# lpylpy0514/VitTracker

Hardware: NVIDIA B200
Metric: tracked frames/sec over B concurrent tracks (higher is better)
Workload: dtype f32

## Files before the change

### vittracker_b200/csrc/vt_block_tc.cu

```cuda
#include "vt_internal.h"
#include "vt_tc.cuh"

namespace vt {

using namespace tc;

#ifdef VT_TC_TRACE
__device__ long long g_tc_trace[2][4096];
__device__ int g_tc_trace_n[2];
#define TC_TRACE(side)                                                                      \
    do {                                                                                    \
        if (blockIdx.x == 0) { int k__ = g_tc_trace_n[side]; if (k__ < 4096) { g_tc_trace[side][k__] = clock64(); g_tc_trace_n[side] = k__ + 1; } } \
    } while (0)
#else
#define TC_TRACE(side) do {} while (0)
#endif

namespace {

#ifndef VT_TC_NS
#define VT_TC_NS 6
#endif
constexpr int kNS = VT_TC_NS;
constexpr int kEpiWarps = 4 * kNS;
constexpr int kEpiThreads = kEpiWarps * 32;
constexpr int kTcThreads = kEpiThreads + 32;
constexpr int kCW = kC / kNS;
constexpr int kQW = 3 * kC / kNS;
constexpr int kHW = kHid / kNS;
static_assert(kNS == 3 || kNS == 6, "column groups");

constexpr uint32_t kColBig = 0;
constexpr uint32_t kColOut = 320;
constexpr uint32_t kColOpa = 368;
constexpr uint32_t kColHA = 0, kColHB = 192;
constexpr uint32_t kColYA = 384, kColYB = 432;

constexpr int kSmWa = 0;
constexpr int kSmX = kSmWa + kTcWaBytes;
constexpr int kKBytes = kN * kC * 2;
constexpr int kSmKhi = kSmX, kSmKlo = kSmX + kKBytes, kSmVhi = kSmX + 2 * kKBytes, kSmVlo = kSmX + 3 * kKBytes;
constexpr int kSmW2hi = kSmX, kSmW2lo = kSmX + 18432;
constexpr int kSmW1 = kSmX + 4 * kKBytes;
constexpr int kSmW1hi = kSmW1, kSmW1lo = kSmW1 + 18432;
constexpr int kSmPar = kSmW1 + 36864;
constexpr int kSmRed = kSmPar + kDepth * kTcParFloats * 4;
constexpr int kSmBar = kSmRed + 6 * kNS * 128 * 4;
constexpr int kSmTmem = kSmBar + 20 * 8;
static_assert(kSmTmem + 16 <= 227 * 1024, "shared memory");
constexpr int kTcSmemBytes = kSmTmem + 16;
static_assert(kTcWbBytes == 2 * 36864 && 36864 <= 4 * kKBytes, "W2 overlays the K/V region");
static_assert(kSmBar % 8 == 0 && kSmX % 128 == 0, "alignment");

constexpr int kPLn1g = 0, kPLn1b = 48, kPBqkv = 96, kPBproj = 240, kPLn2g = 288, kPLn2b = 336, kPBfc1 = 384, kPBfc2 = 576;

__device__ __forceinline__ void epi_bar() { asm volatile("bar.sync 1, %0;" ::"n"(kEpiThreads) : "memory"); }

struct Epi {
    uint32_t tbase;
    uint32_t lane_addr;
    int q, s, lane, row;
    float* red;
    uint64_t *mb_go, *mb_done;
    uint32_t done_ph;

    __device__ __forceinline__ bool active(int t) const { return !(t == 2 && q >= 2); }
    __device__ __forceinline__ uint32_t taddr(uint32_t col) const { return tbase + lane_addr + col; }

    __device__ __forceinline__ void signal(uint64_t* bar, bool wrote_smem) {
        tc_wait_st();
        if (wrote_smem) fence_async_smem();
        tc_fence_before();
        __syncwarp();
        if (lane == 0) mbar_arrive(bar);
    }
    __device__ __forceinline__ void signal_go(bool wrote_smem) { signal(mb_go, wrote_smem); }
    __device__ __forceinline__ void wait_bar(uint64_t* bar, uint32_t& ph) {
        if (threadIdx.x == 0) TC_TRACE(1);
        mbar_wait(bar, ph);
        ph ^= 1;
        tc_fence_after();
        if (threadIdx.x == 0) TC_TRACE(1);
    }
    __device__ __forceinline__ void wait_done() {
        if (threadIdx.x == 0) TC_TRACE(1);
        mbar_wait(mb_done, done_ph);
        done_ph ^= 1;
        tc_fence_after();
        if (threadIdx.x == 0) TC_TRACE(1);
    }

    __device__ __forceinline__ float row_sum(float partial, int arr) {
        float* r = red + arr * (kNS * 128);
        r[s * 128 + row] = partial;
        epi_bar();
        float t = r[row];
#pragma unroll
        for (int g = 1; g < kNS; ++g) t += r[g * 128 + row];
        return t;
    }

    __device__ __forceinline__ void ln(const float (&v)[kCW], const float* g, const float* b, float (&y)[kCW]) {
        float sum = 0.f;
#pragma unroll
        for (int i = 0; i < kCW; ++i) sum += v[i];
        const float mean = row_sum(sum, 0) * (1.f / 48.f);
        float var = 0.f;
#pragma unroll
        for (int i = 0; i < kCW; ++i) { const float d = v[i] - mean; var = fmaf(d, d, var); }
        const float rstd = rsqrtf(row_sum(var, 1) * (1.f / 48.f) + kLnEps);
#pragma unroll
        for (int i = 0; i < kCW; ++i) y[i] = (v[i] - mean) * rstd * g[kCW * s + i] + b[kCW * s + i];
    }

    __device__ __forceinline__ void store_opa(int t, const float (&y)[kCW]) {
        uint32_t hi[kCW / 2], lo[kCW / 2];
#pragma unroll
        for (int j = 0; j < kCW / 2; ++j) split_pack2(y[2 * j], y[2 * j + 1], hi[j], lo[j]);
        tmem_st<kCW / 2>(taddr(kColOpa + 48 * t + (kCW / 2) * s), hi);
        tmem_st<kCW / 2>(taddr(kColOpa + 48 * t + 24 + (kCW / 2) * s), lo);
    }
};

__device__ __forceinline__ float ex2_approx(float x) {
    float y;
    asm("ex2.approx.ftz.f32 %0, %1;" : "=f"(y) : "f"(x));
    return y;
}
__device__ __forceinline__ float rcp_approx(float x) {
    float y;
    asm("rcp.approx.ftz.f32 %0, %1;" : "=f"(y) : "f"(x));
    return y;
}
__device__ __forceinline__ float gelu_erf(float v) {
    const float av = fabsf(v);
    const float t = rcp_approx(fmaf(0.3275911f * 0.70710678118654752f, av, 1.f));
    float p = fmaf(0.5f * 1.061405429f, t, 0.5f * -1.453152027f);
    p = fmaf(p, t, 0.5f * 1.421413741f);
    p = fmaf(p, t, 0.5f * -0.284496736f);
    p = fmaf(p, t, 0.5f * 0.254829592f);
    const float e = ex2_approx(v * (-0.5f * 1.4426950408889634f * v));
    return fmaf(-(av * (p * t)), e, fmaxf(v, 0.f));
}

__device__ __forceinline__ uint64_t f2pack(float lo, float hi) {
    uint64_t r;
    asm("mov.b64 %0, {%1, %2};" : "=l"(r) : "f"(lo), "f"(hi));
    return r;
}
__device__ __forceinline__ void f2unpack(uint64_t v, float& lo, float& hi) { asm("mov.b64 {%0, %1}, %2;" : "=f"(lo), "=f"(hi) : "l"(v)); }
__device__ __forceinline__ uint64_t f2bcast(float c) { return f2pack(c, c); }
__device__ __forceinline__ uint64_t f2fma(uint64_t a, uint64_t b, uint64_t c) {
    uint64_t r;
    asm("fma.rn.f32x2 %0, %1, %2, %3;" : "=l"(r) : "l"(a), "l"(b), "l"(c));
    return r;
}
__device__ __forceinline__ uint64_t f2mul(uint64_t a, uint64_t b) {
    uint64_t r;
    asm("mul.rn.f32x2 %0, %1, %2;" : "=l"(r) : "l"(a), "l"(b));
    return r;
}
__device__ __forceinline__ uint64_t f2add(uint64_t a, uint64_t b) {
    uint64_t r;
    asm("add.rn.f32x2 %0, %1, %2;" : "=l"(r) : "l"(a), "l"(b));
    return r;
}
__device__ __forceinline__ void gelu_erf2(uint64_t v, float& h0, float& h1) {
    float v0, v1;
    f2unpack(v, v0, v1);
    const uint64_t av = f2pack(fabsf(v0), fabsf(v1));
    float d0, d1;
    f2unpack(f2fma(f2bcast(0.3275911f * 0.70710678118654752f), av, f2bcast(1.f)), d0, d1);
    const uint64_t t = f2pack(rcp_approx(d0), rcp_approx(d1));
    uint64_t p = f2fma(f2bcast(-0.5f * 1.061405429f), t, f2bcast(0.5f * 1.453152027f));
    p = f2fma(p, t, f2bcast(-0.5f * 1.421413741f));
    p = f2fma(p, t, f2bcast(0.5f * 0.284496736f));
    p = f2fma(p, t, f2bcast(-0.5f * 0.254829592f));
    float w0, w1;
    f2unpack(f2mul(v, f2mul(f2bcast(-0.5f * 1.4426950408889634f), v)), w0, w1);
    const uint64_t e = f2pack(ex2_approx(w0), ex2_approx(w1));
    f2unpack(f2fma(f2mul(av, f2mul(p, t)), e, f2pack(fmaxf(v0, 0.f), fmaxf(v1, 0.f))), h0, h1);
}

}

template <int kScoresTerms>
__global__ void __launch_bounds__(kTcThreads, 1)
blocks_tc_kernel(const float* __restrict__ tok_z, int z_stride_rows, const float* __restrict__ tok_x, int x_stride_rows,
                 float* __restrict__ out, int n, ModelW w, float* __restrict__ taps, size_t tap_stride) {
    extern __shared__ __align__(128) uint8_t smem[];
    const int tid = threadIdx.x, warp = tid >> 5, lane = tid & 31;
    float* s_par = reinterpret_cast<float*>(smem + kSmPar);
    float* s_red = reinterpret_cast<float*>(smem + kSmRed);
    uint64_t* mb_go = reinterpret_cast<uint64_t*>(smem + kSmBar);
    uint64_t* mb_done = mb_go + 1;
    uint64_t* mb_wa = mb_go + 2;
    uint64_t* mb_wb = mb_go + 3;
    uint64_t* mb_h = mb_go + 4;
    uint64_t* mb_y = mb_go + 6;
    uint64_t* mb_g = mb_go + 8;
    uint64_t* mb_yfree = mb_go + 10;
    uint64_t* mb_w1 = mb_go + 11;
    uint64_t* mb_qd = mb_go + 12;
    uint64_t* mb_pa = mb_go + 15;
    uint64_t* mb_qf = mb_go + 14;
    uint64_t* mb_l1 = mb_go + 16;
    uint32_t* s_tmem = reinterpret_cast<uint32_t*>(smem + kSmTmem);

    if (warp == kEpiWarps) tmem_alloc(s_tmem, 512);
    if (tid == 0) {
        mbar_init(mb_go, kEpiWarps);
        mbar_init(mb_done, 1);
        mbar_init(mb_wa, 1);
        mbar_init(mb_wb, 1);
        mbar_init(mb_w1, 1);
        mbar_init(mb_qd, 1); mbar_init(mb_qd + 1, 1);
        mbar_init(mb_qf, kEpiWarps);
        mbar_init(mb_pa, kEpiWarps);
        for (int t = 0; t < 3; ++t) mbar_init(mb_l1 + t, kEpiWarps);
        mbar_init(mb_h, 1); mbar_init(mb_h + 1, 1);
        mbar_init(mb_y, 1); mbar_init(mb_y + 1, 1);
        mbar_init(mb_g, kEpiWarps); mbar_init(mb_g + 1, kEpiWarps);
        mbar_init(mb_yfree, kEpiWarps);
        mbar_fence_init();
    }
    for (int i = tid; i < kDepth * kTcParFloats; i += kTcThreads) s_par[i] = __ldg(w.tc[i / kTcParFloats].par + i % kTcParFloats);
    tc_fence_before();
    __syncthreads();
    tc_fence_after();
    const uint32_t tbase = __shfl_sync(0xffffffffu, *s_tmem, 0);
    const uint32_t sbase = smem_u32(smem);

    if (warp == kEpiWarps) {
        {
            uint32_t go_ph = 0, wa_ph = 0, wb_ph = 0, w1_ph = 0;
            const uint32_t id48 = instr_desc_f16(128, 48, false), id48mn = instr_desc_f16(128, 48, true);
            const uint32_t id144 = instr_desc_f16(128, 144, false), id160 = instr_desc_f16(128, 160, false);
            const uint32_t id192 = instr_desc_f16(128, 192, false);
            auto wait_go = [&]() { TC_TRACE(0); mbar_wait(mb_go, go_ph); go_ph ^= 1; tc_fence_after(); TC_TRACE(0); };
            auto load_wa = [&](int blk) { bulk_g2s_elect(smem + kSmWa, w.tc[blk].wa, kTcWaBytes, mb_wa); };
            auto load_w1 = [&](int blk) { bulk_g2s_elect(smem + kSmW1, w.tc[blk].wb, 36864, mb_w1); };
            auto load_w2 = [&](int blk) { bulk_g2s_elect(smem + kSmX, w.tc[blk].wb + 36864, 36864, mb_wb); };
            auto gemm_k48 = [&](int t, uint32_t d_col, uint32_t b_hi, uint32_t b_lo, int N, uint32_t idesc) {
                const uint32_t a = tbase + kColOpa + 48 * t;
#pragma unroll
                for (int ks = 0; ks < 3; ++ks) {
                    const uint64_t bh = smem_desc(sbase + b_hi + ks * 2 * N * 16, N * 16, 128);
                    const uint64_t bl = smem_desc(sbase + b_lo + ks * 2 * N * 16, N * 16, 128);
                    mma_ts_elect(tbase + d_col, a + 8 * ks, bh, idesc, ks > 0);
                    mma_ts_elect(tbase + d_col, a + 24 + 8 * ks, bh, idesc, true);
                    mma_ts_elect(tbase + d_col, a + 8 * ks, bl, idesc, true);
                }
            };
            auto qkv = [&](int t, uint32_t d_col) { gemm_k48(t, d_col, kSmWa, kSmWa + 13824, 144, id144); };
            auto fc1 = [&](int t, uint32_t h_col) { gemm_k48(t, h_col, kSmW1hi, kSmW1lo, 192, id192); };
            auto scores_half = [&](int t, int half) {
                const uint32_t a = tbase + kColOpa + 48 * t;
                const uint32_t d = tbase + kColBig + 160 * half;
#pragma unroll
                for (int ks = 0; ks < 3; ++ks) {
                    const uint32_t off = ks * 2 * (kN * 16) + half * 160 * 16;
                    const uint64_t bh = smem_desc(sbase + kSmKhi + off, kN * 16, 128);
                    const uint64_t bl = smem_desc(sbase + kSmKlo + off, kN * 16, 128);
                    mma_ts_elect(d, a + 8 * ks, bh, id160, ks > 0);
                    if (kScoresTerms >= 2) mma_ts_elect(d, a + 24 + 8 * ks, bh, id160, true);
                    if (kScoresTerms >= 3) mma_ts_elect(d, a + 8 * ks, bl, id160, true);
                }
            };
            auto pv = [&](int t, int g0, int g1) {
                const uint32_t d = tbase + kColOpa + 48 * t;
#pragma unroll 5
                for (int g = g0; g < g1; ++g) {
                    const uint32_t a = tbase + kColBig + 16 * g;
                    const uint64_t bh = smem_desc(sbase + kSmVhi + g * 256, 128, (kN / 8) * 128);
                    const uint64_t bl = smem_desc(sbase + kSmVlo + g * 256, 128, (kN / 8) * 128);
                    mma_ts_elect(d, a, bh, id48mn, g > 0);
                    mma_ts_elect(d, a + 8, bh, id48mn, true);
                    mma_ts_elect(d, a, bl, id48mn, true);
                }
            };
            auto fc2 = [&](uint32_t h_col, uint32_t y_col) {
#pragma unroll 4
                for (int g = 0; g < kHid / 16; ++g) {
                    const uint32_t a = tbase + h_col + 16 * g;
                    const uint64_t bh = smem_desc(sbase + kSmW2hi + g * 2 * 48 * 16, 48 * 16, 128);
                    const uint64_t bl = smem_desc(sbase + kSmW2lo + g * 2 * 48 * 16, 48 * 16, 128);
                    mma_ts_elect(tbase + y_col, a, bh, id48, g > 0);
                    mma_ts_elect(tbase + y_col, a + 8, bh, id48, true);
                    mma_ts_elect(tbase + y_col, a, bl, id48, true);
                }
            };
            uint32_t h_ph[2] = {0, 0}, y_ph[2] = {0, 0}, g_ph[2] = {0, 0}, yfree_ph = 0, qf_ph = 0, pa_ph = 0, l1_ph[3] = {0, 0, 0};
            auto wait_on = [&](uint64_t* bar, uint32_t& ph) { TC_TRACE(0); mbar_wait(bar, ph); ph ^= 1; tc_fence_after(); TC_TRACE(0); };
            bool first = true;
            for (int trk = blockIdx.x; trk < n; trk += gridDim.x) {
                const bool last_track = trk + (int)gridDim.x >= n;
                for (int blk = 0; blk < kDepth; ++blk) {
                    if (first) { load_wa(0); load_w1(0); first = false; }
                    wait_on(mb_l1, l1_ph[0]);
                    mbar_wait(mb_wa, wa_ph); wa_ph ^= 1;
                    qkv(0, kColBig); mma_commit_elect(mb_qd);
                    wait_on(mb_l1 + 1, l1_ph[1]); qkv(1, kColBig + 160); mma_commit_elect(mb_qd + 1);
                    wait_on(mb_l1 + 2, l1_ph[2]);
                    wait_on(mb_qf, qf_ph);
                    qkv(2, kColBig); mma_commit_elect(mb_qd);
                    wait_go(); scores_half(0, 0); scores_half(0, 1); mma_commit_elect(mb_done);
#pragma unroll
                    for (int t = 0; t < 3; ++t) {
                        wait_on(mb_pa, pa_ph);
#ifdef VT_TC_LATE_ISSUE
                        wait_go();
                        pv(t, 0, 10);
                        if (t < 2) scores_half(t + 1, 0);
#else
                        pv(t, 0, 10);
                        if (t < 2) scores_half(t + 1, 0);
                        wait_go();
#endif
                        pv(t, 10, 20);
                        if (t < 2) scores_half(t + 1, 1);
                        mma_commit_elect(mb_done);
                    }
                    wait_go(); load_w2(blk);
                    if (!(last_track && blk == kDepth - 1)) load_wa((blk + 1) % kDepth);
                    mbar_wait(mb_w1, w1_ph); w1_ph ^= 1;
                    fc1(0, kColHA); mma_commit_elect(mb_h);
                    wait_on(mb_h, h_ph[0]);
                    fc1(1, kColHB); mma_commit_elect(mb_h + 1);
                    wait_on(mb_g, g_ph[0]);
                    wait_on(mb_h + 1, h_ph[1]);
                    mbar_wait(mb_wb, wb_ph); wb_ph ^= 1;
                    fc2(kColHA, kColYA); mma_commit_elect(mb_y);
                    wait_on(mb_y, y_ph[0]);
                    fc1(2, kColHA); mma_commit_elect(mb_h);
                    wait_on(mb_g + 1, g_ph[1]);
                    wait_on(mb_h, h_ph[0]);
                    if (!(last_track && blk == kDepth - 1)) load_w1((blk + 1) % kDepth);
                    fc2(kColHB, kColYB); mma_commit_elect(mb_y + 1);
                    wait_on(mb_g, g_ph[0]);
                    wait_on(mb_yfree, yfree_ph);
                    fc2(kColHA, kColYA); mma_commit_elect(mb_y);
                    wait_on(mb_y + 1, y_ph[1]);
                    wait_on(mb_y, y_ph[0]);
                }
            }
        }
        __syncwarp();
    } else {
        Epi e;
        e.tbase = tbase; e.q = warp & 3; e.s = warp >> 2; e.lane = lane; e.row = 32 * e.q + lane;
        e.lane_addr = (uint32_t)(32 * e.q) << 16;
        e.red = s_red; e.mb_go = mb_go; e.mb_done = mb_done; e.done_ph = 0;
        const int s = e.s, row = e.row;
        const float scale = 0.14433756729740643f;
        const float kLog2e = 1.4426950408889634f;
        uint32_t h_ph[2] = {0, 0}, y_ph[2] = {0, 0}, qd_ph[2] = {0, 0};
        const int qkv_part = (s * kQW) / 48, qkv_off = (s * kQW) % 48;

        for (int trk = blockIdx.x; trk < n; trk += gridDim.x) {
            float x[3][kCW];
#pragma unroll
            for (int t = 0; t < 3; ++t) {
                const int r = 128 * t + row;
                const float* src = nullptr;
                if (r < kNz) src = tok_z + ((size_t)trk * z_stride_rows + r) * kC + kCW * s;
                else if (r < kN) src = tok_x + ((size_t)trk * x_stride_rows + (r - kNz)) * kC + kCW * s;
#pragma unroll
                for (int i = 0; i < kCW; i += 4) {
                    float4 v = make_float4(0.f, 0.f, 0.f, 0.f);
                    if (src) v = __ldg(reinterpret_cast<const float4*>(src + i));
                    x[t][i] = v.x; x[t][i + 1] = v.y; x[t][i + 2] = v.z; x[t][i + 3] = v.w;
                }
                if (taps && r < kN) {
                    float* tp = taps + ((size_t)trk * kN + r) * kC + kCW * s;
#pragma unroll
                    for (int i = 0; i < kCW; i += 4) *reinterpret_cast<float4*>(tp + i) = make_float4(x[t][i], x[t][i + 1], x[t][i + 2], x[t][i + 3]);
                }
            }

#pragma unroll 1
            for (int blk = 0; blk < kDepth; ++blk) {
                const float* par = s_par + blk * kTcParFloats;

#pragma unroll
                for (int t = 0; t < 3; ++t) {
                    float y[kCW];
                    e.ln(x[t], par + kPLn1g, par + kPLn1b, y);
                    if (e.active(t)) e.store_opa(t, y);
                    e.signal(mb_l1 + t, false);
                }

                auto epi_qkv = [&](int t, uint32_t col) {
                    if (!e.active(t)) return;
                    float v[kQW];
                    {
                        uint32_t r[kQW / 8][8];
#pragma unroll
                        for (int c = 0; c < kQW / 8; ++c) tmem_ld8(e.taddr(col + kQW * s + 8 * c), r[c]);
                        tc_wait_ld();
#pragma unroll
                        for (int c = 0; c < kQW / 8; ++c)
#pragma unroll
                            for (int j = 0; j < 8; ++j) v[8 * c + j] = __uint_as_float(r[c][j]) + par[kPBqkv + kQW * s + 8 * c + j];
                    }
                    const int key = 128 * t + row;
                    if (qkv_part == 0) {
#pragma unroll
                        for (int c = 0; c < kQW / 2; c += 4) {
                            uint32_t hi[4], lo[4];
#pragma unroll
                            for (int j = 0; j < 4; ++j) split_pack2(v[2 * (c + j)] * scale, v[2 * (c + j) + 1] * scale, hi[j], lo[j]);
                            tmem_st4(e.taddr(kColOpa + 48 * t + qkv_off / 2 + c), hi);
                            if (kScoresTerms >= 2) tmem_st4(e.taddr(kColOpa + 48 * t + 24 + qkv_off / 2 + c), lo);
                        }
                    } else {
                        uint8_t* hi_base = smem + (qkv_part == 1 ? kSmKhi : kSmVhi) + key * 16 + (qkv_off / 8) * (kN * 16);
                        uint8_t* lo_base = smem + (qkv_part == 1 ? kSmKlo : kSmVlo) + key * 16 + (qkv_off / 8) * (kN * 16);
#pragma unroll
                        for (int c = 0; c < kQW / 8; ++c) {
                            uint32_t hi[4], lo[4];
#pragma unroll
                            for (int j = 0; j < 4; ++j) split_pack2(v[8 * c + 2 * j], v[8 * c + 2 * j + 1], hi[j], lo[j]);
                            *reinterpret_cast<uint4*>(hi_base + c * (kN * 16)) = make_uint4(hi[0], hi[1], hi[2], hi[3]);
                            if (qkv_part == 2 || kScoresTerms >= 3)
                                *reinterpret_cast<uint4*>(lo_base + c * (kN * 16)) = make_uint4(lo[0], lo[1], lo[2], lo[3]);
                        }
                    }
                };
                e.wait_bar(mb_qd, qd_ph[0]);      epi_qkv(0, kColBig);        e.signal(mb_qf, true);
                e.wait_bar(mb_qd + 1, qd_ph[1]);  epi_qkv(1, kColBig + 160);
                e.wait_bar(mb_qd, qd_ph[0]);      epi_qkv(2, kColBig);        e.signal_go(true);

                auto softmax = [&](int t) {
                    constexpr int kRounds = (20 + kNS - 1) / kNS;
                    constexpr int kRoundsA = (10 + kNS - 1) / kNS;
                    const int my_groups = (20 - s + kNS - 1) / kNS;
                    const uint32_t a0 = e.taddr(kColBig + 16 * s);
                    float m = -INFINITY;
                    if (e.active(t)) {
#pragma unroll
                        for (int k = 0; k < kRounds; ++k) {
                            if (k < my_groups) {
                                uint32_t r[16];
                                tmem_ld16(a0 + 16 * kNS * k, r);
                                tc_wait_ld();
#pragma unroll
                                for (int j = 0; j < 16; ++j) m = fmaxf(m, __uint_as_float(r[j]));
                            }
                        }
                    }
                    float* rm = e.red + ((t & 1) ? 5 : 2) * (kNS * 128);
                    rm[s * 128 + row] = m;
                    epi_bar();
                    m = rm[row];
#pragma unroll
                    for (int g = 1; g < kNS; ++g) m = fmaxf(m, rm[g * 128 + row]);
                    float l = 0.f;
                    const float mb = m * kLog2e;
#pragma unroll
                    for (int k = 0; k < kRounds; ++k) {
                        if (e.active(t) && k < my_groups) {
                            uint32_t r[16];
                            tmem_ld16(a0 + 16 * kNS * k, r);
                            tc_wait_ld();
                            uint32_t hi[8], lo[8];
#ifdef VT_SCALAR_GELU
                            float l0 = 0.f, l1 = 0.f;
#pragma unroll
                            for (int j = 0; j < 8; ++j) {
                                const float p0 = ex2_approx(fmaf(__uint_as_float(r[2 * j]), kLog2e, -mb));
                                const float p1 = ex2_approx(fmaf(__uint_as_float(r[2 * j + 1]), kLog2e, -mb));
                                l0 += p0; l1 += p1;
                                split_pack2(p0, p1, hi[j], lo[j]);
                            }
#else
                            uint64_t l2 = 0ull;
                            const uint64_t nmb2 = f2bcast(-mb);
#pragma unroll
                            for (int j = 0; j < 8; ++j) {
                                float a0, a1;
                                f2unpack(f2fma(f2pack(__uint_as_float(r[2 * j]), __uint_as_float(r[2 * j + 1])), f2bcast(kLog2e), nmb2), a0, a1);
                                const float p0 = ex2_approx(a0), p1 = ex2_approx(a1);
                                l2 = f2add(l2, f2pack(p0, p1));
                                split_pack2(p0, p1, hi[j], lo[j]);
                            }
                            float l0, l1;
                            f2unpack(l2, l0, l1);
#endif
                            l += l0 + l1;
                            tmem_st8(a0 + 16 * kNS * k, hi);
                            tmem_st8(a0 + 16 * kNS * k + 8, lo);
                        }
                        if (k == kRoundsA - 1) e.signal(mb_pa, false);
                    }
                    e.red[(3 + (t & 1)) * (kNS * 128) + s * 128 + row] = l;
                    e.signal_go(false);
                };
                auto epi_out = [&](int t) {
                    epi_bar();
                    const float* rl = e.red + (3 + (t & 1)) * (kNS * 128);
                    float lsum = rl[row];
#pragma unroll
                    for (int g = 1; g < kNS; ++g) lsum += rl[g * 128 + row];
                    const float inv = 1.f / lsum;
                    if (e.active(t)) {
                        uint32_t r[kCW];
                        tmem_ld<kCW>(e.taddr(kColOpa + 48 * t + kCW * s), r);
                        tc_wait_ld();
#pragma unroll
                        for (int j = 0; j < kCW; ++j) x[t][j] += fmaf(__uint_as_float(r[j]), inv, par[kPBproj + kCW * s + j]);
                    }
                    float y[kCW];
                    e.ln(x[t], par + kPLn2g, par + kPLn2b, y);
                    if (e.active(t)) e.store_opa(t, y);
                };
                e.wait_done(); softmax(0);
                e.wait_done(); softmax(1); epi_out(0);
                e.wait_done(); softmax(2); epi_out(1);
                e.wait_done(); epi_out(2); e.signal_go(false);

                auto gelu = [&](int t, uint32_t h_col) {
                    if (!e.active(t)) return;
                    const uint32_t a0 = e.taddr(h_col + kHW * s);
#pragma unroll
                    for (int g = 0; g < kHW / 16; ++g) {
                        uint32_t r[16];
                        tmem_ld16(a0 + 16 * g, r);
                        tc_wait_ld();
                        uint32_t hi[8], lo[8];
#pragma unroll
                        for (int j = 0; j < 8; ++j) {
#ifdef VT_SCALAR_GELU
                            const float h0 = gelu_erf(__uint_as_float(r[2 * j]) + par[kPBfc1 + kHW * s + 16 * g + 2 * j]);
                            const float h1 = gelu_erf(__uint_as_float(r[2 * j + 1]) + par[kPBfc1 + kHW * s + 16 * g + 2 * j + 1]);
#else
                            float h0, h1;
                            gelu_erf2(f2add(f2pack(__uint_as_float(r[2 * j]), __uint_as_float(r[2 * j + 1])),
                                            f2pack(par[kPBfc1 + kHW * s + 16 * g + 2 * j], par[kPBfc1 + kHW * s + 16 * g + 2 * j + 1])), h0, h1);
#endif
                            split_pack2(h0, h1, hi[j], lo[j]);
                        }
                        tmem_st8(a0 + 16 * g, hi);
                        tmem_st8(a0 + 16 * g + 8, lo);
                    }
                };
                auto epi_fc2 = [&](int t, uint32_t y_col) {
                    if (!e.active(t)) return;
                    uint32_t r[kCW];
                    tmem_ld<kCW>(e.taddr(y_col + kCW * s), r);
                    tc_wait_ld();
#pragma unroll
                    for (int j = 0; j < kCW; ++j) x[t][j] += __uint_as_float(r[j]) + par[kPBfc2 + kCW * s + j];
                    const int rr = 128 * t + row;
                    if (taps && rr < kN) {
                        float* tp = taps + (size_t)(blk + 1) * tap_stride + ((size_t)trk * kN + rr) * kC + kCW * s;
#pragma unroll
                        for (int i = 0; i < kCW; i += 4) *reinterpret_cast<float4*>(tp + i) = make_float4(x[t][i], x[t][i + 1], x[t][i + 2], x[t][i + 3]);
                    }
                    if (blk == kDepth - 1 && rr < kN) {
                        float* dst = out + ((size_t)trk * kN + rr) * kC + kCW * s;
#pragma unroll
                        for (int i = 0; i < kCW; i += 4) *reinterpret_cast<float4*>(dst + i) = make_float4(x[t][i], x[t][i + 1], x[t][i + 2], x[t][i + 3]);
                    }
                };
                e.wait_bar(mb_h, h_ph[0]);      gelu(0, kColHA);     e.signal(mb_g, false);
                e.wait_bar(mb_h + 1, h_ph[1]);  gelu(1, kColHB);     e.signal(mb_g + 1, false);
                e.wait_bar(mb_y, y_ph[0]);      epi_fc2(0, kColYA);  e.signal(mb_yfree, false);
                e.wait_bar(mb_h, h_ph[0]);      gelu(2, kColHA);     e.signal(mb_g, false);
                e.wait_bar(mb_y + 1, y_ph[1]);  epi_fc2(1, kColYB);
                e.wait_bar(mb_y, y_ph[0]);      epi_fc2(2, kColYA);
            }
        }
    }

    tc_fence_before();
    __syncthreads();
    if (warp == kEpiWarps) tmem_dealloc(tbase, 512);
}

#ifdef VT_TC_WATCHDOG
extern "C" int vt_tc_watchdog_read(int* rec, int* n) {
    cudaDeviceSynchronize();
    cudaMemcpyFromSymbol(n, tc::g_wd_n, sizeof(int));
    cudaMemcpyFromSymbol(rec, tc::g_wd_rec, sizeof(int) * 256 * 6);
    return 0;
}
#endif

#ifdef VT_TC_TRACE
extern "C" int vt_tc_trace_read(long long* host, int* n) {
    cudaDeviceSynchronize();
    cudaMemcpyFromSymbol(n, g_tc_trace_n, 2 * sizeof(int));
    cudaMemcpyFromSymbol(host, g_tc_trace, sizeof(long long) * 2 * 4096);
    int zero[2] = {0, 0};
    cudaMemcpyToSymbol(g_tc_trace_n, zero, sizeof zero);
    return 0;
}
#endif

int launch_blocks_tc(const float* tok_z, int z_stride_rows, const float* tok_x, int x_stride_rows, float* out, int n,
                     const ModelW& w, float* taps, size_t tap_stride, int num_sms, int scores_terms, cudaStream_t st) {
    if (n <= 0) return 0;
    static DeviceOnce once1, once3;
    if (!ensure_dyn_smem(once1, blocks_tc_kernel<1>, kTcSmemBytes) || !ensure_dyn_smem(once3, blocks_tc_kernel<3>, kTcSmemBytes)) return -1;
    const int grid = n < num_sms ? n : num_sms;
    if (scores_terms == 1) blocks_tc_kernel<1><<<grid, kTcThreads, kTcSmemBytes, st>>>(tok_z, z_stride_rows, tok_x, x_stride_rows, out, n, w, taps, tap_stride);
    else blocks_tc_kernel<3><<<grid, kTcThreads, kTcSmemBytes, st>>>(tok_z, z_stride_rows, tok_x, x_stride_rows, out, n, w, taps, tap_stride);
    return cudaGetLastError() == cudaSuccess ? 1 : -1;
}

}
```

Before: 830,200.

## Skip template-token rows in last block and prefetch next track's inputs

Reorders tokens so search tokens occupy the first two 128-row tiles and template tokens the third. In the final block, when no taps are requested, the template tile's query-side attention, MLP and output are skipped, since only search-token outputs are consumed downstream. The freed time is used to prefetch the next track's inputs, compute its first LayerNorm early and issue its next FC1 weight load. The risk is that template-token outputs in `out` are no longer written for the last block, and the barrier phase bookkeeping becomes more intricate.

```diff
diff --git a/vittracker_b200/csrc/vt_block_tc.cu b/vittracker_b200/csrc/vt_block_tc.cu
--- a/vittracker_b200/csrc/vt_block_tc.cu
+++ b/vittracker_b200/csrc/vt_block_tc.cu
@@ -296,6 +296,8 @@
             for (int trk = blockIdx.x; trk < n; trk += gridDim.x) {
                 const bool last_track = trk + (int)gridDim.x >= n;
                 for (int blk = 0; blk < kDepth; ++blk) {
+                    const bool cut = !taps && blk == kDepth - 1;
+                    const int nt = cut ? 2 : 3;
                     if (first) { load_wa(0); load_w1(0); first = false; }
                     wait_on(mb_l1, l1_ph[0]);
                     mbar_wait(mb_wa, wa_ph); wa_ph ^= 1;
@@ -307,18 +309,19 @@
                     wait_go(); scores_half(0, 0); scores_half(0, 1); mma_commit_elect(mb_done);
 #pragma unroll
                     for (int t = 0; t < 3; ++t) {
+                        if (t >= nt) break;
                         wait_on(mb_pa, pa_ph);
 #ifdef VT_TC_LATE_ISSUE
                         wait_go();
                         pv(t, 0, 10);
-                        if (t < 2) scores_half(t + 1, 0);
+                        if (t + 1 < nt) scores_half(t + 1, 0);
 #else
                         pv(t, 0, 10);
-                        if (t < 2) scores_half(t + 1, 0);
+                        if (t + 1 < nt) scores_half(t + 1, 0);
                         wait_go();
 #endif
                         pv(t, 10, 20);
-                        if (t < 2) scores_half(t + 1, 1);
+                        if (t + 1 < nt) scores_half(t + 1, 1);
                         mma_commit_elect(mb_done);
                     }
                     wait_go(); load_w2(blk);
@@ -329,17 +332,24 @@
                     fc1(1, kColHB); mma_commit_elect(mb_h + 1);
                     wait_on(mb_g, g_ph[0]);
                     wait_on(mb_h + 1, h_ph[1]);
+                    if (cut && !last_track) load_w1(0);
                     mbar_wait(mb_wb, wb_ph); wb_ph ^= 1;
                     fc2(kColHA, kColYA); mma_commit_elect(mb_y);
-                    wait_on(mb_y, y_ph[0]);
-                    fc1(2, kColHA); mma_commit_elect(mb_h);
+                    if (!cut) {
+                        wait_on(mb_y, y_ph[0]);
+                        fc1(2, kColHA); mma_commit_elect(mb_h);
+                    }
                     wait_on(mb_g + 1, g_ph[1]);
-                    wait_on(mb_h, h_ph[0]);
-                    if (!(last_track && blk == kDepth - 1)) load_w1((blk + 1) % kDepth);
+                    if (!cut) {
+                        wait_on(mb_h, h_ph[0]);
+                        if (!(last_track && blk == kDepth - 1)) load_w1((blk + 1) % kDepth);
+                    }
                     fc2(kColHB, kColYB); mma_commit_elect(mb_y + 1);
-                    wait_on(mb_g, g_ph[0]);
-                    wait_on(mb_yfree, yfree_ph);
-                    fc2(kColHA, kColYA); mma_commit_elect(mb_y);
+                    if (!cut) {
+                        wait_on(mb_g, g_ph[0]);
+                        wait_on(mb_yfree, yfree_ph);
+                        fc2(kColHA, kColYA); mma_commit_elect(mb_y);
+                    }
                     wait_on(mb_y + 1, y_ph[1]);
                     wait_on(mb_y, y_ph[0]);
                 }
@@ -357,22 +367,26 @@
         uint32_t h_ph[2] = {0, 0}, y_ph[2] = {0, 0}, qd_ph[2] = {0, 0};
         const int qkv_part = (s * kQW) / 48, qkv_off = (s * kQW) % 48;
 
+        auto token = [&](int t) { return t < 2 ? kNz + 128 * t + row : row; };
+        float x[3][kCW];
+        auto load_x = [&](int tr, int t) {
+            const float* src = nullptr;
+            if (t < 2) src = tok_x + ((size_t)tr * x_stride_rows + 128 * t + row) * kC + kCW * s;
+            else if (e.active(t)) src = tok_z + ((size_t)tr * z_stride_rows + row) * kC + kCW * s;
+#pragma unroll
+            for (int i = 0; i < kCW; i += 4) {
+                float4 v = make_float4(0.f, 0.f, 0.f, 0.f);
+                if (src) v = __ldg(reinterpret_cast<const float4*>(src + i));
+                x[t][i] = v.x; x[t][i + 1] = v.y; x[t][i + 2] = v.z; x[t][i + 3] = v.w;
+            }
+        };
+        bool ahead = false;
         for (int trk = blockIdx.x; trk < n; trk += gridDim.x) {
-            float x[3][kCW];
 #pragma unroll
             for (int t = 0; t < 3; ++t) {
-                const int r = 128 * t + row;
-                const float* src = nullptr;
-                if (r < kNz) src = tok_z + ((size_t)trk * z_stride_rows + r) * kC + kCW * s;
-                else if (r < kN) src = tok_x + ((size_t)trk * x_stride_rows + (r - kNz)) * kC + kCW * s;
-#pragma unroll
-                for (int i = 0; i < kCW; i += 4) {
-                    float4 v = make_float4(0.f, 0.f, 0.f, 0.f);
-                    if (src) v = __ldg(reinterpret_cast<const float4*>(src + i));
-                    x[t][i] = v.x; x[t][i + 1] = v.y; x[t][i + 2] = v.z; x[t][i + 3] = v.w;
-                }
-                if (taps && r < kN) {
-                    float* tp = taps + ((size_t)trk * kN + r) * kC + kCW * s;
+                if (!ahead || t == 1) load_x(trk, t);
+                if (taps && e.active(t)) {
+                    float* tp = taps + ((size_t)trk * kN + token(t)) * kC + kCW * s;
 #pragma unroll
                     for (int i = 0; i < kCW; i += 4) *reinterpret_cast<float4*>(tp + i) = make_float4(x[t][i], x[t][i + 1], x[t][i + 2], x[t][i + 3]);
                 }
@@ -381,9 +395,11 @@
 #pragma unroll 1
             for (int blk = 0; blk < kDepth; ++blk) {
                 const float* par = s_par + blk * kTcParFloats;
+                const bool cut = !taps && blk == kDepth - 1;
 
 #pragma unroll
                 for (int t = 0; t < 3; ++t) {
+                    if (blk == 0 && t == 0 && ahead) continue;
                     float y[kCW];
                     e.ln(x[t], par + kPLn1g, par + kPLn1b, y);
                     if (e.active(t)) e.store_opa(t, y);
@@ -391,7 +407,7 @@
                 }
 
                 auto epi_qkv = [&](int t, uint32_t col) {
-                    if (!e.active(t)) return;
+                    if (!e.active(t) || (cut && t == 2 && qkv_part == 0)) return;
                     float v[kQW];
                     {
                         uint32_t r[kQW / 8][8];
@@ -403,7 +419,7 @@
 #pragma unroll
                             for (int j = 0; j < 8; ++j) v[8 * c + j] = __uint_as_float(r[c][j]) + par[kPBqkv + kQW * s + 8 * c + j];
                     }
-                    const int key = 128 * t + row;
+                    const int key = token(t);
                     if (qkv_part == 0) {
 #pragma unroll
                         for (int c = 0; c < kQW / 2; c += 4) {
@@ -516,8 +532,9 @@
                 };
                 e.wait_done(); softmax(0);
                 e.wait_done(); softmax(1); epi_out(0);
-                e.wait_done(); softmax(2); epi_out(1);
-                e.wait_done(); epi_out(2); e.signal_go(false);
+                e.wait_done(); if (!cut) softmax(2); epi_out(1);
+                if (!cut) { e.wait_done(); epi_out(2); }
+                e.signal_go(false);
 
                 auto gelu = [&](int t, uint32_t h_col) {
                     if (!e.active(t)) return;
@@ -551,13 +568,13 @@
                     tc_wait_ld();
 #pragma unroll
                     for (int j = 0; j < kCW; ++j) x[t][j] += __uint_as_float(r[j]) + par[kPBfc2 + kCW * s + j];
-                    const int rr = 128 * t + row;
-                    if (taps && rr < kN) {
+                    const int rr = token(t);
+                    if (taps) {
                         float* tp = taps + (size_t)(blk + 1) * tap_stride + ((size_t)trk * kN + rr) * kC + kCW * s;
 #pragma unroll
                         for (int i = 0; i < kCW; i += 4) *reinterpret_cast<float4*>(tp + i) = make_float4(x[t][i], x[t][i + 1], x[t][i + 2], x[t][i + 3]);
                     }
-                    if (blk == kDepth - 1 && rr < kN) {
+                    if (blk == kDepth - 1) {
                         float* dst = out + ((size_t)trk * kN + rr) * kC + kCW * s;
 #pragma unroll
                         for (int i = 0; i < kCW; i += 4) *reinterpret_cast<float4*>(dst + i) = make_float4(x[t][i], x[t][i + 1], x[t][i + 2], x[t][i + 3]);
@@ -565,10 +582,23 @@
                 };
                 e.wait_bar(mb_h, h_ph[0]);      gelu(0, kColHA);     e.signal(mb_g, false);
                 e.wait_bar(mb_h + 1, h_ph[1]);  gelu(1, kColHB);     e.signal(mb_g + 1, false);
-                e.wait_bar(mb_y, y_ph[0]);      epi_fc2(0, kColYA);  e.signal(mb_yfree, false);
-                e.wait_bar(mb_h, h_ph[0]);      gelu(2, kColHA);     e.signal(mb_g, false);
+                e.wait_bar(mb_y, y_ph[0]);      epi_fc2(0, kColYA);
+                float y0[kCW];
+                if (cut) {
+                    ahead = trk + (int)gridDim.x < n;
+                    if (ahead) {
+                        load_x(trk + gridDim.x, 0);
+                        load_x(trk + gridDim.x, 2);
+                        e.ln(x[0], s_par + kPLn1g, s_par + kPLn1b, y0);
+                    }
+                }
+                if (!cut) {
+                    e.signal(mb_yfree, false);
+                    e.wait_bar(mb_h, h_ph[0]);  gelu(2, kColHA);     e.signal(mb_g, false);
+                }
                 e.wait_bar(mb_y + 1, y_ph[1]);  epi_fc2(1, kColYB);
-                e.wait_bar(mb_y, y_ph[0]);      epi_fc2(2, kColYA);
+                if (cut && ahead) { e.store_opa(0, y0); e.signal(mb_l1, false); }
+                if (!cut) { e.wait_bar(mb_y, y_ph[0]); epi_fc2(2, kColYA); }
             }
         }
     }
```

Result: no change. 834,000, median of 6 (+0.5%).
